# tomoyoshki/focal

Hardware: AMD Instinct MI355X
Metric: pretrain windows/sec (whole node), FOCAL SW_Transformer (higher is better)
Workload: dtype bf16

## Files before the change

focal_amd/_lib.py:

```python
import ctypes as C
import os

_HERE = os.path.dirname(os.path.abspath(__file__))
LIB_PATH = os.environ.get("FOCAL_HIP_LIB") or os.path.join(_HERE, "libfocal_hip.so")

FOCAL_F32, FOCAL_BF16 = 0, 1
ACT_NONE, ACT_GELU, ACT_RELU_OUT = 0, 1, 2
EPI_NONE, EPI_RESIDUAL, EPI_RELU, EPI_GELU = 0, 1, 2, 3
BN_EVAL, BN_TRAIN, BN_PARTIAL, BN_FINALIZE = 0, 1, 2, 3
BN_SCRATCH_ZEROED = 16
BN_STAT_SLOTS = 16
ABI_VERSION = 14


class DropDesc(C.Structure):
    _fields_ = [("rng", C.c_void_p), ("stream_elem", C.c_uint32), ("p_elem", C.c_float),
                ("stream_path", C.c_uint32), ("p_path", C.c_float), ("rows_per_sample", C.c_int)]


class FFTDesc(C.Structure):
    _fields_ = [(n, C.c_int) for n in ("B", "C", "I", "n", "n1", "n2")]


class AugDesc(C.Structure):
# ... 134 lines not shown
    "focal_pad_patch_embed_ape_ln2_fwd": (C.c_int, [C.POINTER(Embed2Desc), P, P, P, P, P, P, P, P, P, C.c_float, C.c_int, P, P, P]),
    "focal_ape_bwd": (C.c_int, [C.c_int, C.c_int, P, P, P]),
    "focal_ape_add_fwd": (C.c_int, [C.c_int, C.c_int, P, P, P]),
    "focal_layernorm_fwd": (C.c_int, [C.POINTER(LNDesc), P, P, P, P, P, P]),
    "focal_layernorm_bwd": (C.c_int, [C.POINTER(LNDesc), P, P, P, P, P, C.c_int, P, P, P, C.POINTER(DropDesc), P]),
    "focal_mask_cast": (C.c_int, [C.c_int, C.c_int, C.c_int, P, C.POINTER(DropDesc), P, P]),
    "focal_linear_fwd": (C.c_int, [C.POINTER(LinearDesc), P, P, P, P, P, P, P]),
    "focal_linear_resid_ln_fwd": (C.c_int, [C.POINTER(LinearDesc), P, P, P, P, P, P, P, C.c_float, P, P, P]),
    "focal_linear_resid_ln_supported": (C.c_int, [C.c_int, C.c_int, C.c_int]),
    "focal_linear_bwd_data": (C.c_int, [C.POINTER(LinearDesc), P, P, P, P, P]),
    "focal_linear_bwd_data_ln": (C.c_int, [C.POINTER(LinearDesc), P, P, P, P, P, P, P, P, P, C.POINTER(DropDesc), P]),
    "focal_linear_bwd_data_ln_supported": (C.c_int, [C.c_int, C.c_int, C.c_int]),
    "focal_linear_bwd_weight": (C.c_int, [C.POINTER(LinearDesc), P, P, P, P, P]),
    "focal_linear_bwd_weight_workgroups": (C.c_int, [C.POINTER(LinearDesc)]),
    "focal_linear_bwd_weight_kernel": (C.c_int, [C.POINTER(LinearDesc)]),
    "focal_linear_bwd_weight_group": (C.c_int, [C.c_int, C.c_int, C.POINTER(DwProblem), P]),
    "focal_linear_bwd_weight_group_supported": (C.c_int, [C.c_int, C.c_int, C.c_int, C.c_int]),
    "focal_linear_bwd_weight_group_workgroups": (C.c_int, [C.c_int, C.c_int, C.POINTER(DwProblem)]),
    "focal_linear_bwd_weight_group_f32": (C.c_int, [C.c_int, C.c_int, C.POINTER(DwProblem), C.c_int, C.c_void_p]),
    "focal_linear_bwd_weight_group_f32_workgroups": (C.c_int, [C.c_int, C.c_int, C.POINTER(DwProblem), C.c_int]),
    "focal_linear_bwd_weight_group_kind": (C.c_int, [C.c_int, C.c_int, C.c_int, C.c_int]),
    "focal_mlp_supported": (C.c_int, [C.c_int, C.c_int, C.c_int]),
    "focal_mlp_fwd": (C.c_int, [C.POINTER(MlpDesc), P, P, P, P, P, P, P, P, P, P, P, P, P]),
    "focal_mlp_bwd": (C.c_int, [C.POINTER(MlpDesc), P, P, P, P, P, P, P, P, P, P, P, P, P, P, P, C.POINTER(DropDesc), P, P, P, P, P]),
    "focal_mlp_bwd_partials_floats": (C.c_long, [C.POINTER(MlpDesc)]),
    "focal_mlp_proj_supported": (C.c_int, [C.c_int, C.c_int, C.c_int]),
    "focal_mlp_proj_fwd": (C.c_int, [C.POINTER(MlpDesc), P, P, P, P, C.POINTER(DropDesc), P, P, P, P, P, P, P, P, P, P, P, P, P, P, P, P]),
    "focal_mlp_wide_supported": (C.c_int, [C.c_int, C.c_int, C.c_int]),
    "focal_mlp_wide_fwd": (C.c_int, [C.POINTER(MlpDesc), P, P, P, P, P, P, P, P, P, P, P, P, P, P]),
    "focal_mlp_wide_proj_supported": (C.c_int, [C.c_int, C.c_int, C.c_int]),
# ... 90 lines not shown
```

focal_amd/csrc/gemm.hpp:

```cpp
#pragma once
#include <stdlib.h>
#include <type_traits>
#include "common.hpp"

enum GemmPro { PRO_NONE = 0, PRO_GELU = 1, PRO_MASK = 2, PRO_CONV = 3 };
enum GemmEpi { EPI_STORE = 0, EPI_RESID = 1, EPI_MUL_AUX = 2, EPI_RELU = 3, EPI_RELU_BWD = 4, EPI_ATOMIC = 5, EPI_GELU_FWD = 6,
               EPI_RESID_LN = 7,
               EPI_LN_BWD = 8,
               EPI_STORE_STATS = 9 };

struct MaskParams {
  const uint32_t* seed;
  uint32_t stream_elem;
  float p_elem;
  uint32_t stream_path;
  float p_path;
  int rows_per_sample;
  int ncols;
};

struct GemmParams {
  int M, N, K;
  const void* A; long lda; long strideA;
  const void* B; long ldb; long strideB;
// ... 284 lines not shown
__global__ __launch_bounds__(256) void focal_dw_tail_group_kernel(const DwTailGroup g) {
  using TA = float;
  using TB = float;
  using TC = float;
  constexpr bool TRA = true, TRB = true;
  constexpr int PROA = PRO_NONE, PROB = PRO_NONE, EPI = EPI_ATOMIC, BM = 64, BN = 64, BKM = 2;
  int pi = 0;
#pragma unroll
  for (int q = 0; q < DW_TAIL_MAX - 1; ++q) pi += (q < g.n - 1 && (int)blockIdx.x >= g.wg_end[q]) ? 1 : 0;
  const int start = pi > 0 ? g.wg_end[pi - 1] : 0;
  const GemmParams& p = g.p[pi];
  const int block = (int)blockIdx.x - start, nblocks = g.wg_end[pi] - start;
#include "gemm_body.inc"
}

static inline void focal_dw_plan(int M, int N, long rows, int target, int* bm_out, int* bn_out, int* splits_out) {
  const int bm = 64, bn = 64;
  const long tiles = (long)((M + bm - 1) / bm) * ((N + bn - 1) / bn);
  const long target_wg = target > 0 ? target : 512;
  long splits = (target_wg + tiles - 1) / tiles;
  const long min_rows = 256;
  const long max_splits = (rows + min_rows - 1) / min_rows;
  if (splits > max_splits) splits = max_splits;
  if (splits < 1) splits = 1;
  *bm_out = bm; *bn_out = bn; *splits_out = (int)splits;
}

static inline bool focal_dw_ring_shape(int M, int N, long rows) {
  return M % 64 == 0 && N % 64 == 0 && rows % 64 == 0 && rows >= 64;
}
// ... 3 lines not shown
  int pairs = (splits + 1) / 2;
  if (tiles <= 256 && tiles * pairs > 256) pairs = 256 / tiles;
  return pairs < 1 ? 1 : pairs;
}

struct GemmSpec {
  int compute;
  int a_dtype, b_dtype, c_dtype;
  bool tra, trb;
  int proA, proB, epi;
};
int focal_launch_gemm_bf16(const GemmSpec& s, const GemmParams& p, hipStream_t stream);
int focal_launch_gemm_f32(const GemmSpec& s, const GemmParams& p, hipStream_t stream);
int focal_launch_dw_tail_bf16(const DwTailGroup& g, hipStream_t stream);
int focal_launch_dw_tail_f32(const DwTailGroup& g, hipStream_t stream);
static inline int focal_launch_gemm(const GemmSpec& s, const GemmParams& p, hipStream_t stream) {
  if ((p.epi.p_elem > 0.f || p.proA.p_elem > 0.f || p.proB.p_elem > 0.f) && ((long)p.M >= (1L << 24) || (long)p.K >= (1L << 24) || (long)p.N >= (1L << 24))) {
    focal_set_error("gemm: a dimension beyond 2^24 with an element mask (MaskEval indexes elements with 24-bit multiplies)");
    return FOCAL_EUNSUPPORTED;
  }
  return s.compute == FOCAL_F32 ? focal_launch_gemm_f32(s, p, stream) : focal_launch_gemm_bf16(s, p, stream);
}
```

focal_amd/csrc/gemm_bf16.hip:

```cpp
#include <stdlib.h>
#include <type_traits>
#include "gemm_ring.hpp"
#include "gemm_dw_ring.hpp"
#define GEMM_CT bf16_t
#define GEMM_TAIL_FN focal_launch_dw_tail_bf16
#define GEMM_FN focal_launch_gemm_bf16
#include "gemm_dispatch.inc"
```

focal_amd/csrc/gemm_body.inc:

```
  using Cfg = GemmCfg<CT>;
  constexpr int BK = Cfg::BK * BKM, KI = Cfg::KI;
  using StA = OperandStage<CT, TA, TRA, PROA, BM, BKM>;
  using StB = OperandStage<CT, TB, TRB, PROB, BN, BKM>;
  using FA = FragLoad<CT, TRA, StA::PITCH>;
  using FB = FragLoad<CT, TRB, StB::PITCH>;
  constexpr int WGN = (BN <= 64) ? 1 : 2, WGM = 4 / WGN;
  constexpr int WR = BM / WGM, WC = BN / WGN;
  constexpr int TM = WR / 16, TN = WC / 16;

  constexpr int OPER_BYTES = (StA::LDS_ELEMS + StB::LDS_ELEMS) * (int)sizeof(CT);
  constexpr int EPI_RP = (WC > 64 || WR < 32) ? 16 : 32;
  constexpr int STAGE_BYTES = 4 * EPI_RP * (WC + 4) * 4;
  constexpr int LDS_BYTES = OPER_BYTES > STAGE_BYTES ? OPER_BYTES : STAGE_BYTES;
  __shared__ __attribute__((aligned(16))) char lds_raw[LDS_BYTES];
  CT* lds = reinterpret_cast<CT*>(lds_raw);
  CT* ldsA = lds;
  CT* ldsB = lds + StA::LDS_ELEMS;

  const int tid = threadIdx.x, lane = tid & 63, wave = tid >> 6;
  const int wm = wave / WGN, wn = wave % WGN;
  const int tiles_n = (p.N + BN - 1) / BN, tiles_m = (p.M + BM - 1) / BM;
  const int ntiles = tiles_m * tiles_n;
  const int logical = xcd_remap(block, nblocks);
  const int tile = logical % ntiles, z = logical / ntiles;
  const int m0 = (tile / tiles_n) * BM, n0 = (tile % tiles_n) * BN;
  const int bz = z / p.splits, sp = z % p.splits;

  const TA* A = reinterpret_cast<const TA*>(p.A) + (long)bz * p.strideA;
  const TB* B = reinterpret_cast<const TB*>(p.B) + (long)bz * p.strideB;
  TC* C = reinterpret_cast<TC*>(p.C) + (long)bz * p.strideC;

  const int KT = (p.K + BK - 1) / BK;
  const int kt_per = (KT + p.splits - 1) / p.splits;
  const int kt0 = sp * kt_per;
  const int kt1 = min(KT, kt0 + kt_per);
  const int k_end = min(p.K, kt1 * BK);

  MaskEval meA, meB, meE;
  if (PROA != PRO_NONE) meA.init(p.proA);
  if (PROB != PRO_NONE) meB.init(p.proB);
  if (EPI == EPI_RESID || EPI == EPI_GELU_FWD || EPI == EPI_RESID_LN) meE.init(p.epi);

  f32x4 acc[TM][TN];
#pragma unroll
  for (int i = 0; i < TM; ++i)
#pragma unroll
    for (int j = 0; j < TN; ++j) acc[i][j] = f32x4{0.f, 0.f, 0.f, 0.f};

  float csum[8] = {0.f, 0.f, 0.f, 0.f, 0.f, 0.f, 0.f, 0.f};
  const bool do_colsum = TRA && (p.colsumA != nullptr) && (n0 == 0);

  constexpr bool PF2 = false;
  StA sa0, sa1;
  StB sb0, sb1;
  auto step = [&](StA& sa, StB& sb, int kt, int kt_next) {
    if (TRA && do_colsum) sa.template store<true>(ldsA, m0, kt * BK, tid, meA, csum);
// ... 109 lines not shown
        const int row = rr + lane / LPR;
        const int m = mbase + row;
        if (m >= p.M || n >= p.N) continue;
        float v[CPL];
        loadN<CPL>(stage + row * WPITCH + c, v);
#pragma unroll
        for (int e = 0; e < CPL; ++e) v[e] += bias[e];
        TC* dst = C + (long)m * p.ldc + n;
        if (EPI == EPI_STORE) {
          storeN<CPL>(dst, v);
        } else if (EPI == EPI_STORE_STATS) {
          storeN<CPL>(dst, v);
          if constexpr (CPL == 4) {
#pragma unroll
            for (int e = 0; e < 4; ++e) { st_s[e] += v[e]; st_q[e] += v[e] * v[e]; }
          }
        } else if (EPI == EPI_RESID) {
          float r[CPL];
          loadN<CPL>(p.resid + (long)m * p.ldr + n, r);
          const float rowm = meE.row_mult(m);
#pragma unroll
          for (int e = 0; e < CPL; ++e) v[e] = r[e] + v[e] * rowm * meE.elem_mult(m, n + e);
          storeN<CPL>(dst, v);
        } else if (EPI == EPI_RESID_LN) {
          float r[CPL];
          loadN<CPL>(p.resid + (long)m * p.ldr + n, r);
          const float rowm = meE.row_mult(m);
#pragma unroll
          for (int e = 0; e < CPL; ++e) v[e] = r[e] + v[e] * rowm * meE.elem_mult(m, n + e);
          storeN<CPL>(dst, v);
// ... 117 lines not shown
```

focal_amd/csrc/gemm_dispatch.inc:

```

#define GEMM_LAUNCH(BM_, BN_, BKM_)                                                                                         \
  do {                                                                                                                      \
    dim3 grid(ceil_div(p.M, BM_) * ceil_div(p.N, BN_) * nz);                                                                \
    focal_note_kernel("focal_gemm_kernel<%s, trA=%d, trB=%d, proA=%d, proB=%d, epi=%d, %dx%d>", sizeof(CT) == 2 ? "bf16" : "f32", (int)TRA, (int)TRB, PA, PB, EPI, BM_, BN_); \
    FOCAL_LAUNCH((focal_gemm_kernel<CT, TA, TB, TC, TRA, TRB, PA, PB, EPI, BM_, BN_, BKM_>), grid, dim3(256), 0, stream, p); \
  } while (0)

template <typename CT, typename TA, typename TB, typename TC, bool TRA, bool TRB, int PA, int PB, int EPI>
static int launch_dw(GemmParams p, long rows, hipStream_t stream) {
  int bm, bn, splits;
  focal_dw_plan(p.M, p.N, rows, p.dw_target, &bm, &bn, &splits);
  p.splits = splits;
  if constexpr (std::is_same<CT, bf16_t>::value && std::is_same<TA, bf16_t>::value && std::is_same<TB, bf16_t>::value &&
                PA == PRO_NONE && PB == PRO_NONE) {
    const bool aligned = ((uintptr_t)p.A % 16 == 0) && ((uintptr_t)p.B % 16 == 0) && (p.lda % 8 == 0) && (p.ldb % 8 == 0);
    if (aligned && p.batch == 1 && bm == 64 && bn == 64 && focal_dw_ring_shape(p.M, p.N, rows)) {
      hipError_t e;
      if (p.splits >= 2) {
        p.splits = focal_dw_ring_pairs(p.M, p.N, p.splits);
        focal_note_kernel("focal_dw_ring_kernel<64, 4, 2>");
        e = focal_launch_dw_ring<64, 4, 2>(p, stream);
      } else {
        focal_note_kernel("focal_dw_ring_kernel<64, 4, 1>");
        e = focal_launch_dw_ring<64, 4, 1>(p, stream);
// ... 99 lines not shown
          focal_set_error("gemm (pipelined, LayerNorm epilogue): launch failed: %s", hipGetErrorString(e));
          return FOCAL_EHIP;
        }
        return FOCAL_OK;
      }
    }
    if (p.N != 64 || p.splits != 1 || p.batch != 1) {
      focal_set_error("gemm: the residual + LayerNorm epilogue needs N == 64, or bf16 operands with N == 128 / 256 and K %% 64 == 0 (got N = %d, K = %d)", p.N, p.K);
      return FOCAL_EUNSUPPORTED;
    }
    const int nz = 1;
    GEMM_LAUNCH(64, 64, 1);
    FOCAL_LAUNCH_CHECK();
    return FOCAL_OK;
  }
  const long min_wg = 512;
  const long z = (long)p.batch * p.splits;
  const int nz = p.batch * p.splits;
  bool narrow_n = (p.N % 128 != 0) || (p.N < 128);
  bool small_m = (p.M % 128 != 0 && p.M < 1024) || (p.M <= 256);
  if (!small_m && !narrow_n && (long)ceil_div(p.M, 128) * ceil_div(p.N, 128) * z < min_wg) narrow_n = true;
  if (!small_m && narrow_n && (long)ceil_div(p.M, 128) * ceil_div(p.N, 64) * z < min_wg) small_m = true;
  if (!std::is_same<CT, float>::value && p.K <= 1024) small_m = true;
  if (!narrow_n && !small_m) GEMM_LAUNCH(128, 128, 1);
  else if (!small_m) GEMM_LAUNCH(128, 64, 1);
  else GEMM_LAUNCH(64, 64, 1);
  FOCAL_LAUNCH_CHECK();
  return FOCAL_OK;
}

#define GEMM_TRY(AF32, BF32, CF32, TRA_, TRB_, PA_, PB_, EPI_)                                                          \
  if (s.a_dtype == ((AF32) ? FOCAL_F32 : ct_code) && s.b_dtype == ((BF32) ? FOCAL_F32 : ct_code) &&                     \
      s.c_dtype == ((CF32) ? FOCAL_F32 : ct_code) && s.tra == (TRA_) && s.trb == (TRB_) && s.proA == (PA_) &&            \
      s.proB == (PB_) && s.epi == (EPI_))                                                                               \
    return launch_tiles<GEMM_CT, std::conditional<(AF32), float, GEMM_CT>::type,                                        \
                        std::conditional<(BF32), float, GEMM_CT>::type, std::conditional<(CF32), float, GEMM_CT>::type, \
                        (TRA_), (TRB_), (PA_), (PB_), (EPI_)>(p, stream);

int GEMM_FN(const GemmSpec& s, const GemmParams& p, hipStream_t stream) {
  const int ct_code = std::is_same<GEMM_CT, float>::value ? FOCAL_F32 : FOCAL_BF16;
// ... 12 lines not shown
  GEMM_TRY(true, false, true, false, true, PRO_NONE, PRO_NONE, EPI_RELU_BWD)
  GEMM_TRY(true, false, true, false, true, PRO_NONE, PRO_NONE, EPI_STORE)
  GEMM_TRY(false, false, true, true, true, PRO_NONE, PRO_NONE, EPI_ATOMIC)
  GEMM_TRY(true, false, true, true, true, PRO_MASK, PRO_NONE, EPI_ATOMIC)
  GEMM_TRY(true, true, true, true, true, PRO_NONE, PRO_NONE, EPI_ATOMIC)
  GEMM_TRY(false, false, true, false, false, PRO_CONV, PRO_NONE, EPI_STORE)
  GEMM_TRY(false, false, true, false, false, PRO_CONV, PRO_NONE, EPI_STORE_STATS)
  GEMM_TRY(false, false, true, false, false, PRO_CONV, PRO_NONE, EPI_RESID)
  GEMM_TRY(false, false, true, true, true, PRO_NONE, PRO_CONV, EPI_ATOMIC)
  focal_set_error("gemm: unsupported combination a=%d b=%d c=%d trA=%d trB=%d proA=%d proB=%d epi=%d (compute %d)",
                  s.a_dtype, s.b_dtype, s.c_dtype, (int)s.tra, (int)s.trb, s.proA, s.proB, s.epi, ct_code);
  return FOCAL_EUNSUPPORTED;
}
#undef GEMM_TRY

int GEMM_TAIL_FN(const DwTailGroup& g, hipStream_t stream) {
  if (g.n <= 0) return FOCAL_OK;
  focal_note_kernel("focal_dw_tail_group_kernel<%s>", sizeof(GEMM_CT) == 2 ? "bf16" : "f32");
  FOCAL_LAUNCH((focal_dw_tail_group_kernel<GEMM_CT>), dim3(g.wg_end[g.n - 1]), dim3(256), 0, stream, g);
  FOCAL_LAUNCH_CHECK();
  return FOCAL_OK;
}
```

focal_amd/csrc/gemm_f32.hip:

```cpp
#include <stdlib.h>
#include <type_traits>
#include "gemm_ring.hpp"
#include "gemm_dw_ring.hpp"
#define GEMM_CT float
#define GEMM_TAIL_FN focal_launch_dw_tail_f32
#define GEMM_FN focal_launch_gemm_f32
#include "gemm_dispatch.inc"
```

focal_amd/csrc/linear.hip:

```cpp
#include <stdlib.h>
#include "gemm.hpp"
#include "gemm_dw_group.hpp"
#include "gemm_dw_ring.hpp"
#include "gemm_ring.hpp"

static MaskParams to_mask(const focal_drop_desc& d, int ncols) {
  MaskParams m;
  m.seed = d.rng;
  m.stream_elem = d.stream_elem;
  m.p_elem = d.p_elem;
  m.stream_path = d.stream_path;
  m.p_path = d.p_path;
  m.rows_per_sample = d.rows_per_sample;
  m.ncols = ncols;
  return m;
}
static MaskParams no_mask() {
  MaskParams m;
  memset(&m, 0, sizeof(m));
  return m;
}

static int check_desc(const focal_linear_desc* d) {
  FOCAL_CHECK_ARG(d != nullptr, "linear: null descriptor");
// ... 202 lines not shown
  if (ring && splits >= 2) splits = focal_dw_ring_pairs(d->N, d->K, splits);
  *wgs = ((d->N + bm - 1) / bm) * ((d->K + bn - 1) / bn) * splits;
  return true;
}

extern "C" int focal_linear_bwd_weight_workgroups(const focal_linear_desc* d) {
  int kernel, wgs;
  return dw_launch_plan(d, &kernel, &wgs) ? wgs : 0;
}

extern "C" int focal_linear_bwd_weight_kernel(const focal_linear_desc* d) {
  int kernel, wgs;
  return dw_launch_plan(d, &kernel, &wgs) ? kernel : 0;
}

static bool dw_group_fits(const focal_dw_problem& q) {
  return q.M > 0 && q.N > 0 && q.K > 0 && q.M % 64 == 0 && q.N % 128 == 0 && q.K % 128 == 0 && q.dy && q.x && q.dw &&
         ((uintptr_t)q.dy % 16 == 0) && ((uintptr_t)q.x % 16 == 0) && ((uintptr_t)q.dw % 16 == 0);
}

extern "C" int focal_linear_bwd_weight_group_supported(int dtype, int M, int N, int K) {
  return dtype == FOCAL_BF16 && M > 0 && M % 64 == 0 && N % 128 == 0 && K % 128 == 0;
}

static int dw_group_build(int dtype, int n, const focal_dw_problem* probs, DwGroupParams* gp, int* wgs) {
  FOCAL_CHECK_ARG(dtype == FOCAL_BF16, "linear_bwd_weight_group: bf16 operands only (dtype %d)", dtype);
  FOCAL_CHECK_ARG(n >= 1 && n <= DWG_MAX_PROBLEMS && probs, "linear_bwd_weight_group: 1 .. %d problems (got %d)", DWG_MAX_PROBLEMS, n);
  memset(gp, 0, sizeof(*gp));
  gp->nprob = n;
  for (int i = 0; i < n; ++i) {
// ... 120 lines not shown
```

focal_amd/ops.py:

```python
import ctypes as C
import math
import os

import torch

from . import _lib
from ._lib import (ACT_GELU, ACT_NONE, ACT_RELU_OUT, EPI_GELU, EPI_NONE, EPI_RELU, EPI_RESIDUAL, FOCAL_BF16, FOCAL_F32,
                   AdamWDesc, AttnDesc, BNDesc, ConvDesc, ConvInDesc, DropDesc, Embed2Desc, EmbedDesc, FFTDesc, GRUDesc, LinearDesc,
                   LNDesc, LossDesc, MlpDesc, check)

_TORCH2CODE = {torch.float32: FOCAL_F32, torch.bfloat16: FOCAL_BF16}
_CODE2TORCH = {v: k for k, v in _TORCH2CODE.items()}


def code(dtype):
    return _TORCH2CODE[dtype]


def torch_dtype(c):
    return _CODE2TORCH[c]


def _stream():
    return torch.cuda.current_stream().cuda_stream
# ... 474 lines not shown
    return bool(_lib.load().focal_linear_bwd_data_ln_supported(dtype_code, N, K))


def linear_bwd_data_ln(d, dy, w, ln_x, ln_stats, ln_gamma, g, dgamma, dbeta, g_masked=None, mask=None):
    _need_cuda(dy, w, ln_x, ln_stats, ln_gamma, g, dgamma, dbeta, g_masked)
    if g_masked is not None:
        mask = mask or NO_DROP
    check(_lib.load().focal_linear_bwd_data_ln(C.byref(d), _p(dy), _p(w), _p(ln_x), _p(ln_stats), _p(ln_gamma), _p(g), _p(dgamma), _p(dbeta),
                                               _p(g_masked), C.byref(mask) if mask is not None else None, _stream()))


def linear_bwd_weight(d, dy, x, dw, dbias):
    check(_lib.load().focal_linear_bwd_weight(C.byref(d), _p(dy), _p(x), _p(dw), _p(dbias), _stream()))


def dw_group_supported(dtype_code, M, N, K):
    return bool(_lib.load().focal_linear_bwd_weight_group_supported(dtype_code, M, N, K))


def dw_group_kind(dtype_code, M, N, K):
    return int(_lib.load().focal_linear_bwd_weight_group_kind(dtype_code, M, N, K))


def _dw_problems(items, exclusive):
    arr = (_lib.DwProblem * len(items))()
    for i, (dy, x, dw, db) in enumerate(items):
        _need_cuda(dy, x, dw, db)
        arr[i] = _lib.DwProblem(_p(dy), _p(x), _p(dw), _p(db), dy.shape[0], dy.shape[1], x.shape[1], 1 if exclusive else 0)
    return arr

# ... 583 lines not shown
```

focal_amd/src/models/SW_Transformer.py:

```python
import os
import sys

import torch
import torch.nn as nn

_ROOT = os.path.abspath(os.path.join(os.path.dirname(__file__), "..", "..", ".."))
if _ROOT not in sys.path:
    sys.path.insert(0, _ROOT)

from focal_amd import runtime
from focal_amd.backbone import HipBackbone, run_stage
from focal_amd.head_engine import ClassifierHead
from focal_amd.loc_engine import LocFusionStage, run_loc_stage
from focal_amd.swin_engine import ProjectorHead, SwinModEncoder
from input_utils.padding_utils import get_padded_size
from models.FusionModules import LocContextLayer, TransformerFusionBlock
from models.SwinModules import BasicLayer, PatchEmbed, PatchMerging


class SW_Transformer(HipBackbone):
    def __init__(self, args) -> None:
        super().__init__()
        self.args = args
        self.config = args.dataset_config["SW_Transformer"]
        self.modalities = args.dataset_config["modality_names"]
        self.locations = args.dataset_config["location_names"]
        self.num_segments = args.dataset_config["num_segments"]
        self.drop_rate = self.config["dropout_ratio"]
        self.attn_drop_rate = self.config["attn_drop_rate"]
# ... 71 lines not shown
            self.mod_projectors[mod] = nn.Sequential(nn.Linear(cfg["loc_out_channels"], out_dim), nn.ReLU(),
                                                     nn.Linear(out_dim, out_dim))
        self.mod_fusion_layers = TransformerFusionBlock(cfg["loc_out_channels"], cfg["loc_head_num"],
                                                        cfg["dropout_ratio"], cfg["dropout_ratio"])
        self.sample_dim = cfg["loc_out_channels"]
        n_cls = dcfg[self.args.task]["num_classes"]
        if self.args.train_mode == "supervised" or cfg["pretrained_head"] == "linear":
            self.class_layer = nn.Sequential(nn.Linear(self.sample_dim, n_cls))
        else:
            self.class_layer = nn.Sequential(nn.Linear(self.sample_dim, cfg["fc_dim"]), nn.GELU(), nn.Linear(cfg["fc_dim"], n_cls))
        M = len(self.modalities)
        self._encoders = {(loc, mod): SwinModEncoder(self, loc, mod, li * M + mi)
                          for li, loc in enumerate(self.locations) for mi, mod in enumerate(self.modalities)}
        self._loc_stages = ({mod: LocFusionStage(self, mod, mi) for mi, mod in enumerate(self.modalities)}
                            if len(self.locations) > 1 else {})
        self._heads = {mod: ProjectorHead(self, mod) for mod in self.modalities}
        self._class_head = ClassifierHead(self, "mod_fusion_layers", cfg["loc_head_num"], cfg["dropout_ratio"])

    def forward_encoder(self, freq_x, class_head=True, proj_head=False, defer_join=False):
        if class_head:
            return self.forward_classifier(freq_x)
        loc = self.locations[0]
        view = self._fwd_calls
        self._fwd_calls = (self._fwd_calls + 1) & 0xFFFF
        dev = next(self.parameters()).device
        if dev.type != "cuda":
            from focal_amd._lib import FocalHipError
            raise FocalHipError("the FOCAL HIP path needs the model on a ROCm device (no CPU fallback)")
        cur = torch.cuda.current_stream(dev)
        out = {}
        self.arena()
# ... 47 lines not shown
```

focal_amd/swin_engine.py:

```python
import os
from typing import NamedTuple

import torch

from . import ops
from ._lib import ACT_GELU, ACT_NONE, EPI_GELU, EPI_NONE, EPI_RESIDUAL


def tail_fp32(bb, which="mod_in"):
    if bb.compute_dtype == torch.float32:
        return False
    sel = os.environ.get("FOCAL_TAIL_FP32", "projector")
    return sel == "both" or sel == which


def tail_weight(bb, ar, name, which="mod_in"):
    return ar.master(name) if tail_fp32(bb, which) else ar.operand(name)


class BlockPlan(NamedTuple):
    attn_qkv: bool
    mlp: str
    proj: str
    next_ln: bool
# ... 205 lines not shown
        pool = self.__dict__.setdefault("_mlp_ws", {})
        n = ops.mlp_bwd_partials_floats(d_mlp)
        ws = pool.get((n, dev))
        if ws is None:
            ws = pool[(n, dev)] = torch.empty(n, dtype=torch.float32, device=dev)
        return ws

    def backward(self, saved, dfeat):
        bb, ar = self.bb, self.bb.arena()
        ct = bb.compute_dtype
        dev = dfeat.device
        if dfeat.dtype != torch.float32 or not dfeat.is_contiguous():
            dfeat = dfeat.float().contiguous()
        pin, d_in, xf = saved["pin"], saved["d_in"], saved["x_final"]
        d_in_b = ops.linear_desc(d_in.dtype, d_in.M, d_in.N, d_in.K, d_in.x_dtype, d_in.y_dtype)
        ops.linear_bwd_weight(d_in_b, dfeat, xf, ar.g(f"{pin}.weight"), ar.g(f"{pin}.bias"))
        g = torch.empty_like(xf)
        ops.linear_bwd_data(d_in_b, dfeat, tail_weight(bb, ar, f"{pin}.weight"), None, g)
        blocks = saved["blocks"]
        last = blocks[-1]
        gm = ops.mask_cast(g.view(last["M"], last["C"]), last["d_fc2"].out_drop, ct)
        stop = 0
        if getattr(bb, "split_backward", False) and saved["merges"] and saved.get("embed") is None:
            stop = max(m["after_block"] for m in saved["merges"])
        state = dict(g=g, gm=gm, next=len(blocks) - 1)
        self._backward_blocks(saved, state, stop)
        if stop > 0:
            saved["_resume"] = state
            bb.pending_backward.append((self, saved, torch.cuda.current_stream(dev)))
            return
        self._backward_tail(saved, state)

    def backward_rest(self, saved):
        state = saved.pop("_resume")
        self._backward_blocks(saved, state, 0)
        self._backward_tail(saved, state)
# ... 147 lines not shown
        z = torch.empty(B, E, dtype=torch.float32, device=feat.device)
        ops.linear_fwd(d2, h, tail_weight(bb, ar, f"{self.pre}.2.weight", "projector"), ar.master(f"{self.pre}.2.bias"), None, z)
        return z, dict(feat=feat, h=h, d0=d0, d2=d2)

    def backward(self, saved, dz):
        ar = self.bb.arena()
        if dz.dtype != torch.float32 or not dz.is_contiguous():
            dz = dz.float().contiguous()
        ops.linear_bwd_weight(saved["d2"], dz, saved["h"], ar.g(f"{self.pre}.2.weight"), ar.g(f"{self.pre}.2.bias"))
        dh = torch.empty_like(saved["h"])
        ops.linear_bwd_data(saved["d2"], dz, tail_weight(self.bb, ar, f"{self.pre}.2.weight", "projector"), saved["h"], dh)
        ops.linear_bwd_weight(saved["d0"], dh, saved["feat"], ar.g(f"{self.pre}.0.weight"), ar.g(f"{self.pre}.0.bias"))
        dfeat = torch.empty_like(saved["feat"])
        ops.linear_bwd_data(saved["d0"], dh, tail_weight(self.bb, ar, f"{self.pre}.0.weight", "projector"), None, dfeat)
        return dfeat
```

include/focal_hip.h:

```cpp
#ifndef FOCAL_HIP_H
#define FOCAL_HIP_H

#include <stddef.h>
#include <stdint.h>

#ifdef __cplusplus
extern "C" {
#endif

#define FOCAL_ABI_VERSION 14

enum { FOCAL_OK = 0, FOCAL_EINVAL = -1, FOCAL_EUNSUPPORTED = -2, FOCAL_EWORKSPACE = -3, FOCAL_EHIP = -4 };
enum { FOCAL_F32 = 0, FOCAL_BF16 = 1 };

int focal_abi_version(void);
const char* focal_last_kernel(void);
const char* focal_last_error(void);

enum { FOCAL_TRACE_DISPATCH = 1, FOCAL_TRACE_EVENTS = 2 };
typedef struct {
  char kernel[384];
  unsigned grid[3], block[3];
  void* stream;
  float us;
// ... 113 lines not shown
int focal_linear_fwd(const focal_linear_desc* d, const void* x, const void* w, const float* bias, const float* resid,
                     void* y, void* act_grad, void* stream);
int focal_linear_resid_ln_fwd(const focal_linear_desc* d, const void* x, const void* w, const float* bias, const float* resid,
                              float* y, const float* gamma, const float* beta, float eps, void* y_ln, float* stats, void* stream);
int focal_linear_resid_ln_supported(int dtype, int N, int K);
int focal_linear_bwd_data(const focal_linear_desc* d, const void* dy, const void* w, const void* x, void* dx,
                          void* stream);
int focal_linear_bwd_data_ln(const focal_linear_desc* d, const void* dy, const void* w, const float* ln_x, const float* ln_stats,
                             const float* ln_gamma, float* g, float* dgamma, float* dbeta, void* g_masked, const focal_drop_desc* mask,
                             void* stream);
int focal_linear_bwd_data_ln_supported(int dtype, int N, int K);
int focal_linear_bwd_weight(const focal_linear_desc* d, const void* dy, const void* x, float* dw, float* dbias,
                            void* stream);
int focal_linear_bwd_weight_workgroups(const focal_linear_desc* d);
int focal_linear_bwd_weight_kernel(const focal_linear_desc* d);

#define FOCAL_DW_GROUP_MAX_PROBLEMS 20
typedef struct {
  const void* dy; const void* x; float* dw; float* dbias;
  int M, N, K;
  int exclusive;
} focal_dw_problem;
int focal_linear_bwd_weight_group(int dtype, int n, const focal_dw_problem* problems, void* stream);
int focal_linear_bwd_weight_group_supported(int dtype, int M, int N, int K);
int focal_linear_bwd_weight_group_kind(int dtype, int M, int N, int K);
int focal_linear_bwd_weight_group_workgroups(int dtype, int n, const focal_dw_problem* problems);
int focal_linear_bwd_weight_group_f32(int compute, int n, const focal_dw_problem* problems, int workgroups, void* stream);
int focal_linear_bwd_weight_group_f32_workgroups(int compute, int n, const focal_dw_problem* problems, int workgroups);

typedef struct { int dtype; int M, C, hidden; focal_drop_desc drop_hidden, drop_out; float ln_eps; } focal_mlp_desc;
// ... 150 lines not shown
```

Baseline: 51540.

## Fuse tail linear weight- and data-gradient GEMMs into one paired launch with mask-cast epilogue

Adds a combined kernel that runs the weight-gradient GEMM (split-K atomic) and the data-gradient GEMM in one grid, with blocks partitioned between the two, sharing one LDS buffer. A new epilogue writes dx and also the dropout-masked cast copy, which removes the separate mask_cast pass. It is used for the encoder's final projection backward and for the projector head's two linears. This cuts kernel launches and lets the two small GEMMs fill the GPU together, at the cost of a larger shared LDS allocation that may lower occupancy.

```diff
diff --git a/focal_amd/_lib.py b/focal_amd/_lib.py
--- a/focal_amd/_lib.py
+++ b/focal_amd/_lib.py
@@ -172,6 +172,9 @@
     "focal_linear_bwd_weight": (C.c_int, [C.POINTER(LinearDesc), P, P, P, P, P]),
     "focal_linear_bwd_weight_workgroups": (C.c_int, [C.POINTER(LinearDesc)]),
     "focal_linear_bwd_weight_kernel": (C.c_int, [C.POINTER(LinearDesc)]),
+    "focal_linear_bwd_pair_supported": (C.c_int, [C.POINTER(LinearDesc), C.c_int]),
+    "focal_linear_bwd_pair_workgroups": (C.c_int, [C.POINTER(LinearDesc)]),
+    "focal_linear_bwd_pair": (C.c_int, [C.POINTER(LinearDesc), P, P, P, P, P, P, P, C.c_int, C.POINTER(DropDesc), C.c_int, P]),
     "focal_linear_bwd_weight_group": (C.c_int, [C.c_int, C.c_int, C.POINTER(DwProblem), P]),
     "focal_linear_bwd_weight_group_supported": (C.c_int, [C.c_int, C.c_int, C.c_int, C.c_int]),
     "focal_linear_bwd_weight_group_workgroups": (C.c_int, [C.c_int, C.c_int, C.POINTER(DwProblem)]),
diff --git a/focal_amd/csrc/gemm.hpp b/focal_amd/csrc/gemm.hpp
--- a/focal_amd/csrc/gemm.hpp
+++ b/focal_amd/csrc/gemm.hpp
@@ -7,7 +7,8 @@
 enum GemmEpi { EPI_STORE = 0, EPI_RESID = 1, EPI_MUL_AUX = 2, EPI_RELU = 3, EPI_RELU_BWD = 4, EPI_ATOMIC = 5, EPI_GELU_FWD = 6,
                EPI_RESID_LN = 7,
                EPI_LN_BWD = 8,
-               EPI_STORE_STATS = 9 };
+               EPI_STORE_STATS = 9,
+               EPI_STORE_MASKCAST = 10 };
 
 struct MaskParams {
   const uint32_t* seed;
@@ -322,6 +323,52 @@
 #include "gemm_body.inc"
 }
 
+struct TailPair { int dw_wgs; GemmParams dw, dx; };
+template <typename CT, bool TRA, bool TRB, int BM, int BN, int BKM> constexpr int gemm_body_lds_bytes() {
+  constexpr int WGN = (BN <= 64) ? 1 : 2, WGM = 4 / WGN, WR = BM / WGM, WC = BN / WGN;
+  constexpr int oper = (OperandStage<CT, CT, TRA, PRO_NONE, BM, BKM>::LDS_ELEMS + OperandStage<CT, CT, TRB, PRO_NONE, BN, BKM>::LDS_ELEMS) * (int)sizeof(CT);
+  constexpr int stage = 4 * ((WC > 64 || WR < 32) ? 16 : 32) * (WC + 4) * 4;
+  return oper > stage ? oper : stage;
+}
+template <typename CT, int EPI_DX>
+__global__ __launch_bounds__(256) void focal_tail_pair_kernel(const TailPair g) {
+  constexpr int DW_LDS = gemm_body_lds_bytes<CT, true, true, 64, 64, 2>(), DX_LDS = gemm_body_lds_bytes<CT, false, true, 64, 64, 1>();
+  constexpr int GEMM_BODY_SHARED_LDS_BYTES = DW_LDS > DX_LDS ? DW_LDS : DX_LDS;
+  __shared__ __attribute__((aligned(16))) char pair_lds[GEMM_BODY_SHARED_LDS_BYTES];
+#define GEMM_BODY_SHARED_LDS pair_lds
+  if ((int)blockIdx.x < g.dw_wgs) {
+    using TA = float;
+    using TB = float;
+    using TC = float;
+    constexpr bool TRA = true, TRB = true;
+    constexpr int PROA = PRO_NONE, PROB = PRO_NONE, EPI = EPI_ATOMIC, BM = 64, BN = 64, BKM = 2;
+    const GemmParams& p = g.dw;
+    const int block = (int)blockIdx.x, nblocks = g.dw_wgs;
+#include "gemm_body.inc"
+  } else {
+    using TA = float;
+    using TB = CT;
+    using TC = float;
+    constexpr bool TRA = false, TRB = true;
+    constexpr int PROA = PRO_NONE, PROB = PRO_NONE, EPI = EPI_DX, BM = 64, BN = 64, BKM = 1;
+    const GemmParams& p = g.dx;
+    const int block = (int)blockIdx.x - g.dw_wgs, nblocks = (int)gridDim.x - g.dw_wgs;
+#include "gemm_body.inc"
+  }
+#undef GEMM_BODY_SHARED_LDS
+}
+
+static inline void focal_tile_plan(bool f32_compute, int M, int N, int K, long z, int* bm_out, int* bn_out) {
+  const long min_wg = 512;
+  bool narrow_n = (N % 128 != 0) || (N < 128);
+  bool small_m = (M % 128 != 0 && M < 1024) || (M <= 256);
+  if (!small_m && !narrow_n && (long)((M + 127) / 128) * ((N + 127) / 128) * z < min_wg) narrow_n = true;
+  if (!small_m && narrow_n && (long)((M + 127) / 128) * ((N + 63) / 64) * z < min_wg) small_m = true;
+  if (!f32_compute && K <= 1024) small_m = true;
+  *bm_out = small_m ? 64 : 128;
+  *bn_out = (!narrow_n && !small_m) ? 128 : 64;
+}
+
 static inline void focal_dw_plan(int M, int N, long rows, int target, int* bm_out, int* bn_out, int* splits_out) {
   const int bm = 64, bn = 64;
   const long tiles = (long)((M + bm - 1) / bm) * ((N + bn - 1) / bn);
@@ -355,6 +402,8 @@
 int focal_launch_gemm_f32(const GemmSpec& s, const GemmParams& p, hipStream_t stream);
 int focal_launch_dw_tail_bf16(const DwTailGroup& g, hipStream_t stream);
 int focal_launch_dw_tail_f32(const DwTailGroup& g, hipStream_t stream);
+int focal_launch_tail_pair_bf16(const TailPair& g, int epi_dx, int dx_wgs, hipStream_t stream);
+int focal_launch_tail_pair_f32(const TailPair& g, int epi_dx, int dx_wgs, hipStream_t stream);
 static inline int focal_launch_gemm(const GemmSpec& s, const GemmParams& p, hipStream_t stream) {
   if ((p.epi.p_elem > 0.f || p.proA.p_elem > 0.f || p.proB.p_elem > 0.f) && ((long)p.M >= (1L << 24) || (long)p.K >= (1L << 24) || (long)p.N >= (1L << 24))) {
     focal_set_error("gemm: a dimension beyond 2^24 with an element mask (MaskEval indexes elements with 24-bit multiplies)");
diff --git a/focal_amd/csrc/gemm_bf16.hip b/focal_amd/csrc/gemm_bf16.hip
--- a/focal_amd/csrc/gemm_bf16.hip
+++ b/focal_amd/csrc/gemm_bf16.hip
@@ -4,5 +4,6 @@
 #include "gemm_dw_ring.hpp"
 #define GEMM_CT bf16_t
 #define GEMM_TAIL_FN focal_launch_dw_tail_bf16
+#define GEMM_PAIR_FN focal_launch_tail_pair_bf16
 #define GEMM_FN focal_launch_gemm_bf16
 #include "gemm_dispatch.inc"
diff --git a/focal_amd/csrc/gemm_body.inc b/focal_amd/csrc/gemm_body.inc
--- a/focal_amd/csrc/gemm_body.inc
+++ b/focal_amd/csrc/gemm_body.inc
@@ -12,7 +12,12 @@
   constexpr int EPI_RP = (WC > 64 || WR < 32) ? 16 : 32;
   constexpr int STAGE_BYTES = 4 * EPI_RP * (WC + 4) * 4;
   constexpr int LDS_BYTES = OPER_BYTES > STAGE_BYTES ? OPER_BYTES : STAGE_BYTES;
+#ifdef GEMM_BODY_SHARED_LDS
+  static_assert(LDS_BYTES <= GEMM_BODY_SHARED_LDS_BYTES, "the including kernel's shared buffer is too small for this body");
+  char* const lds_raw = GEMM_BODY_SHARED_LDS;
+#else
   __shared__ __attribute__((aligned(16))) char lds_raw[LDS_BYTES];
+#endif
   CT* lds = reinterpret_cast<CT*>(lds_raw);
   CT* ldsA = lds;
   CT* ldsB = lds + StA::LDS_ELEMS;
@@ -39,7 +44,7 @@
   MaskEval meA, meB, meE;
   if (PROA != PRO_NONE) meA.init(p.proA);
   if (PROB != PRO_NONE) meB.init(p.proB);
-  if (EPI == EPI_RESID || EPI == EPI_GELU_FWD || EPI == EPI_RESID_LN) meE.init(p.epi);
+  if (EPI == EPI_RESID || EPI == EPI_GELU_FWD || EPI == EPI_RESID_LN || EPI == EPI_STORE_MASKCAST) meE.init(p.epi);
 
   f32x4 acc[TM][TN];
 #pragma unroll
@@ -179,6 +184,16 @@
           if constexpr (CPL == 4) {
 #pragma unroll
             for (int e = 0; e < 4; ++e) { st_s[e] += v[e]; st_q[e] += v[e] * v[e]; }
+          }
+        } else if (EPI == EPI_STORE_MASKCAST) {
+          storeN<CPL>(dst, v);
+          if constexpr (CPL == 4) {
+            const long off = (long)m * p.ldc + n;
+            const uint32_t trow = (uint32_t)(off / meE.ncols);
+            const float pm = meE.on_p ? drop_mult(meE.p, meE.rps > 1 ? __umulhi(trow, meE.rps_magic) : trow) : 1.0f;
+#pragma unroll
+            for (int e = 0; e < CPL; ++e) v[e] *= meE.on_e ? pm * drop_mult(meE.e, (uint32_t)off + e) : pm;
+            storeN<CPL>(reinterpret_cast<CT*>(p.aux_out) + off, v);
           }
         } else if (EPI == EPI_RESID) {
           float r[CPL];
diff --git a/focal_amd/csrc/gemm_dispatch.inc b/focal_amd/csrc/gemm_dispatch.inc
--- a/focal_amd/csrc/gemm_dispatch.inc
+++ b/focal_amd/csrc/gemm_dispatch.inc
@@ -137,16 +137,11 @@
     FOCAL_LAUNCH_CHECK();
     return FOCAL_OK;
   }
-  const long min_wg = 512;
-  const long z = (long)p.batch * p.splits;
   const int nz = p.batch * p.splits;
-  bool narrow_n = (p.N % 128 != 0) || (p.N < 128);
-  bool small_m = (p.M % 128 != 0 && p.M < 1024) || (p.M <= 256);
-  if (!small_m && !narrow_n && (long)ceil_div(p.M, 128) * ceil_div(p.N, 128) * z < min_wg) narrow_n = true;
-  if (!small_m && narrow_n && (long)ceil_div(p.M, 128) * ceil_div(p.N, 64) * z < min_wg) small_m = true;
-  if (!std::is_same<CT, float>::value && p.K <= 1024) small_m = true;
-  if (!narrow_n && !small_m) GEMM_LAUNCH(128, 128, 1);
-  else if (!small_m) GEMM_LAUNCH(128, 64, 1);
+  int bm, bn;
+  focal_tile_plan(std::is_same<CT, float>::value, p.M, p.N, p.K, (long)p.batch * p.splits, &bm, &bn);
+  if (bm == 128 && bn == 128) GEMM_LAUNCH(128, 128, 1);
+  else if (bm == 128) GEMM_LAUNCH(128, 64, 1);
   else GEMM_LAUNCH(64, 64, 1);
   FOCAL_LAUNCH_CHECK();
   return FOCAL_OK;
@@ -189,6 +184,20 @@
 }
 #undef GEMM_TRY
 
+int GEMM_PAIR_FN(const TailPair& g, int epi_dx, int dx_wgs, hipStream_t stream) {
+  const dim3 grid(g.dw_wgs + dx_wgs);
+  focal_note_kernel("focal_tail_pair_kernel<%s, dX epi=%d>", sizeof(GEMM_CT) == 2 ? "bf16" : "f32", epi_dx);
+  if (epi_dx == EPI_STORE) FOCAL_LAUNCH((focal_tail_pair_kernel<GEMM_CT, EPI_STORE>), grid, dim3(256), 0, stream, g);
+  else if (epi_dx == EPI_RELU_BWD) FOCAL_LAUNCH((focal_tail_pair_kernel<GEMM_CT, EPI_RELU_BWD>), grid, dim3(256), 0, stream, g);
+  else if (epi_dx == EPI_STORE_MASKCAST) FOCAL_LAUNCH((focal_tail_pair_kernel<GEMM_CT, EPI_STORE_MASKCAST>), grid, dim3(256), 0, stream, g);
+  else {
+    focal_set_error("tail pair: no data-gradient epilogue %d", epi_dx);
+    return FOCAL_EUNSUPPORTED;
+  }
+  FOCAL_LAUNCH_CHECK();
+  return FOCAL_OK;
+}
+
 int GEMM_TAIL_FN(const DwTailGroup& g, hipStream_t stream) {
   if (g.n <= 0) return FOCAL_OK;
   focal_note_kernel("focal_dw_tail_group_kernel<%s>", sizeof(GEMM_CT) == 2 ? "bf16" : "f32");
diff --git a/focal_amd/csrc/gemm_f32.hip b/focal_amd/csrc/gemm_f32.hip
--- a/focal_amd/csrc/gemm_f32.hip
+++ b/focal_amd/csrc/gemm_f32.hip
@@ -4,5 +4,6 @@
 #include "gemm_dw_ring.hpp"
 #define GEMM_CT float
 #define GEMM_TAIL_FN focal_launch_dw_tail_f32
+#define GEMM_PAIR_FN focal_launch_tail_pair_f32
 #define GEMM_FN focal_launch_gemm_f32
 #include "gemm_dispatch.inc"
diff --git a/focal_amd/csrc/linear.hip b/focal_amd/csrc/linear.hip
--- a/focal_amd/csrc/linear.hip
+++ b/focal_amd/csrc/linear.hip
@@ -240,6 +240,81 @@
   return dw_launch_plan(d, &kernel, &wgs) ? kernel : 0;
 }
 
+static bool pair_fits(const focal_linear_desc* d, int gm_dtype) {
+  if (d == nullptr || d->M <= 0 || d->N <= 0 || d->K <= 0) return false;
+  if (d->dtype != FOCAL_F32 && d->dtype != FOCAL_BF16) return false;
+  const int ec = d->dtype == FOCAL_BF16 ? 8 : 4;
+  if (d->N % ec != 0 || d->K % ec != 0) return false;
+  if (d->x_dtype != FOCAL_F32 || d->y_dtype != FOCAL_F32 || d->epilogue == FOCAL_EPI_RESIDUAL) return false;
+  if (d->act_in != FOCAL_ACT_NONE && d->act_in != FOCAL_ACT_RELU_OUT) return false;
+  if (gm_dtype >= 0 && (gm_dtype != d->dtype || d->act_in != FOCAL_ACT_NONE)) return false;
+  int bm, bn;
+  focal_tile_plan(d->dtype == FOCAL_F32, d->M, d->K, d->N, 1, &bm, &bn);
+  return bm == 64 && bn == 64;
+}
+
+extern "C" int focal_linear_bwd_pair_supported(const focal_linear_desc* d, int gm_dtype) { return pair_fits(d, gm_dtype) ? 1 : 0; }
+
+static int pair_dx_workgroups(const focal_linear_desc* d) { return ceil_div(d->M, 64) * ceil_div(d->K, 64); }
+
+extern "C" int focal_linear_bwd_pair_workgroups(const focal_linear_desc* d) {
+  if (!pair_fits(d, -1)) return 0;
+  return focal_linear_bwd_weight_workgroups(d) + pair_dx_workgroups(d);
+}
+
+extern "C" int focal_linear_bwd_pair(const focal_linear_desc* d, const void* dy, const void* w, const void* x, void* dx, float* dw,
+                                     float* dbias, void* gm, int gm_dtype, const focal_drop_desc* mask, int mask_cols, void* stream) {
+  if (int rc = check_desc(d)) return rc;
+  FOCAL_CHECK_ARG(dy && w && x && dx && dw, "linear_bwd_pair: null tensor");
+  if (!pair_fits(d, gm ? gm_dtype : -1)) {
+    focal_set_error("linear_bwd_pair: unsupported layer (dtype %d, M=%d N=%d K=%d, x/y dtype %d/%d, act_in %d, epilogue %d, masked copy dtype %d): "
+                    "fp32 activations, no output mask, a 64 x 64 data-gradient tile and a masked copy in the compute type only",
+                    d->dtype, d->M, d->N, d->K, d->x_dtype, d->y_dtype, d->act_in, d->epilogue, gm ? gm_dtype : -1);
+    return FOCAL_EUNSUPPORTED;
+  }
+  FOCAL_CHECK_ARG(gm || !mask, "linear_bwd_pair: mask without a masked copy");
+  if (gm) {
+    FOCAL_CHECK_ARG(mask_cols > 0 && mask_cols % 4 == 0 && ((long)d->M * d->K) % mask_cols == 0,
+                    "linear_bwd_pair: dx [%d, %d] is not a whole number of %d-column token rows", d->M, d->K, mask_cols);
+    const long token_rows = (long)d->M * d->K / mask_cols;
+    FOCAL_CHECK_ARG((long)d->M * d->K < (1L << 32) && (!mask || mask->rows_per_sample <= 1 || token_rows * (long)mask->rows_per_sample < (1L << 32)),
+                    "linear_bwd_pair: %ld token rows exceed the mask's 32-bit arithmetic", token_rows);
+  }
+  TailPair g;
+  memset(&g, 0, sizeof(g));
+  {
+    GemmParams& p = g.dw;
+    p.M = d->N; p.N = d->K; p.K = d->M;
+    p.A = dy; p.lda = d->N;
+    p.B = x; p.ldb = d->K;
+    p.C = dw; p.ldc = d->K;
+    p.batch = 1; p.alpha = 1.f;
+    p.dw_target = d->dw_workgroups;
+    p.colsumA = dbias;
+    int bm, bn, splits;
+    focal_dw_plan(p.M, p.N, p.K, p.dw_target, &bm, &bn, &splits);
+    p.splits = splits;
+    g.dw_wgs = ceil_div(p.M, bm) * ceil_div(p.N, bn) * splits;
+  }
+  {
+    GemmParams& p = g.dx;
+    p.M = d->M; p.N = d->K; p.K = d->N;
+    p.A = dy; p.lda = d->N;
+    p.B = w; p.ldb = d->K;
+    p.C = dx; p.ldc = d->K;
+    p.batch = 1; p.splits = 1; p.alpha = 1.f;
+    p.aux = x; p.ldaux = d->K;
+    p.aux_out = gm;
+    focal_drop_desc dd;
+    memset(&dd, 0, sizeof(dd));
+    if (mask) dd = *mask;
+    p.epi = gm ? to_mask(dd, mask_cols) : no_mask();
+  }
+  const int epi = gm ? EPI_STORE_MASKCAST : d->act_in == FOCAL_ACT_RELU_OUT ? EPI_RELU_BWD : EPI_STORE;
+  return d->dtype == FOCAL_F32 ? focal_launch_tail_pair_f32(g, epi, pair_dx_workgroups(d), (hipStream_t)stream)
+                               : focal_launch_tail_pair_bf16(g, epi, pair_dx_workgroups(d), (hipStream_t)stream);
+}
+
 static bool dw_group_fits(const focal_dw_problem& q) {
   return q.M > 0 && q.N > 0 && q.K > 0 && q.M % 64 == 0 && q.N % 128 == 0 && q.K % 128 == 0 && q.dy && q.x && q.dw &&
          ((uintptr_t)q.dy % 16 == 0) && ((uintptr_t)q.x % 16 == 0) && ((uintptr_t)q.dw % 16 == 0);
diff --git a/focal_amd/ops.py b/focal_amd/ops.py
--- a/focal_amd/ops.py
+++ b/focal_amd/ops.py
@@ -512,6 +512,23 @@
     check(_lib.load().focal_linear_bwd_weight(C.byref(d), _p(dy), _p(x), _p(dw), _p(dbias), _stream()))
 
 
+def linear_bwd_pair_supported(d, gm_dtype=None):
+    return bool(_lib.load().focal_linear_bwd_pair_supported(C.byref(d), -1 if gm_dtype is None else code(gm_dtype)))
+
+
+def linear_bwd_pair_workgroups(d):
+    return int(_lib.load().focal_linear_bwd_pair_workgroups(C.byref(d)))
+
+
+def linear_bwd_pair(d, dy, w, x, dx, dw, dbias, gm=None, mask=None):
+    _need_cuda(dy, w, x, dx, dw, dbias, gm)
+    if gm is not None and gm.numel() != dx.numel():
+        raise _lib.FocalHipError("linear_bwd_pair: gm must cover dx")
+    check(_lib.load().focal_linear_bwd_pair(C.byref(d), _p(dy), _p(w), _p(x), _p(dx), _p(dw), _p(dbias), _p(gm),
+                                            -1 if gm is None else code(gm.dtype), C.byref(mask) if mask is not None else None,
+                                            0 if gm is None else gm.shape[-1], _stream()))
+
+
 def dw_group_supported(dtype_code, M, N, K):
     return bool(_lib.load().focal_linear_bwd_weight_group_supported(dtype_code, M, N, K))
 
diff --git a/focal_amd/src/models/SW_Transformer.py b/focal_amd/src/models/SW_Transformer.py
--- a/focal_amd/src/models/SW_Transformer.py
+++ b/focal_amd/src/models/SW_Transformer.py
@@ -12,7 +12,7 @@
 from focal_amd.backbone import HipBackbone, run_stage
 from focal_amd.head_engine import ClassifierHead
 from focal_amd.loc_engine import LocFusionStage, run_loc_stage
-from focal_amd.swin_engine import ProjectorHead, SwinModEncoder
+from focal_amd.swin_engine import SwinModEncoder, SwinProjectorHead
 from input_utils.padding_utils import get_padded_size
 from models.FusionModules import LocContextLayer, TransformerFusionBlock
 from models.SwinModules import BasicLayer, PatchEmbed, PatchMerging
@@ -114,7 +114,7 @@
                           for li, loc in enumerate(self.locations) for mi, mod in enumerate(self.modalities)}
         self._loc_stages = ({mod: LocFusionStage(self, mod, mi) for mi, mod in enumerate(self.modalities)}
                             if len(self.locations) > 1 else {})
-        self._heads = {mod: ProjectorHead(self, mod) for mod in self.modalities}
+        self._heads = {mod: SwinProjectorHead(self, mod) for mod in self.modalities}
         self._class_head = ClassifierHead(self, "mod_fusion_layers", cfg["loc_head_num"], cfg["dropout_ratio"])
 
     def forward_encoder(self, freq_x, class_head=True, proj_head=False, defer_join=False):
diff --git a/focal_amd/swin_engine.py b/focal_amd/swin_engine.py
--- a/focal_amd/swin_engine.py
+++ b/focal_amd/swin_engine.py
@@ -243,12 +243,17 @@
             dfeat = dfeat.float().contiguous()
         pin, d_in, xf = saved["pin"], saved["d_in"], saved["x_final"]
         d_in_b = ops.linear_desc(d_in.dtype, d_in.M, d_in.N, d_in.K, d_in.x_dtype, d_in.y_dtype)
-        ops.linear_bwd_weight(d_in_b, dfeat, xf, ar.g(f"{pin}.weight"), ar.g(f"{pin}.bias"))
         g = torch.empty_like(xf)
-        ops.linear_bwd_data(d_in_b, dfeat, tail_weight(bb, ar, f"{pin}.weight"), None, g)
         blocks = saved["blocks"]
         last = blocks[-1]
-        gm = ops.mask_cast(g.view(last["M"], last["C"]), last["d_fc2"].out_drop, ct)
+        if ops.linear_bwd_pair_supported(d_in_b, ct):
+            gm = torch.empty(last["M"], last["C"], dtype=ct, device=dev)
+            ops.linear_bwd_pair(d_in_b, dfeat, tail_weight(bb, ar, f"{pin}.weight"), xf.view(d_in_b.M, d_in_b.K), g, ar.g(f"{pin}.weight"),
+                                ar.g(f"{pin}.bias"), gm=gm, mask=last["d_fc2"].out_drop)
+        else:
+            ops.linear_bwd_weight(d_in_b, dfeat, xf, ar.g(f"{pin}.weight"), ar.g(f"{pin}.bias"))
+            ops.linear_bwd_data(d_in_b, dfeat, tail_weight(bb, ar, f"{pin}.weight"), None, g)
+            gm = ops.mask_cast(g.view(last["M"], last["C"]), last["d_fc2"].out_drop, ct)
         stop = 0
         if getattr(bb, "split_backward", False) and saved["merges"] and saved.get("embed") is None:
             stop = max(m["after_block"] for m in saved["merges"])
@@ -426,3 +431,20 @@
         dfeat = torch.empty_like(saved["feat"])
         ops.linear_bwd_data(saved["d0"], dh, tail_weight(self.bb, ar, f"{self.pre}.0.weight", "projector"), None, dfeat)
         return dfeat
+
+
+class SwinProjectorHead(ProjectorHead):
+
+    def backward(self, saved, dz):
+        ar = self.bb.arena()
+        d2, d0 = saved["d2"], saved["d0"]
+        if not (ops.linear_bwd_pair_supported(d2) and ops.linear_bwd_pair_supported(d0)):
+            return super().backward(saved, dz)
+        if dz.dtype != torch.float32 or not dz.is_contiguous():
+            dz = dz.float().contiguous()
+        w = lambda i: tail_weight(self.bb, ar, f"{self.pre}.{i}.weight", "projector")
+        dh = torch.empty_like(saved["h"])
+        ops.linear_bwd_pair(d2, dz, w(2), saved["h"], dh, ar.g(f"{self.pre}.2.weight"), ar.g(f"{self.pre}.2.bias"))
+        dfeat = torch.empty_like(saved["feat"])
+        ops.linear_bwd_pair(d0, dh, w(0), saved["feat"], dfeat, ar.g(f"{self.pre}.0.weight"), ar.g(f"{self.pre}.0.bias"))
+        return dfeat
diff --git a/include/focal_hip.h b/include/focal_hip.h
--- a/include/focal_hip.h
+++ b/include/focal_hip.h
@@ -151,6 +151,10 @@
                             void* stream);
 int focal_linear_bwd_weight_workgroups(const focal_linear_desc* d);
 int focal_linear_bwd_weight_kernel(const focal_linear_desc* d);
+int focal_linear_bwd_pair_supported(const focal_linear_desc* d, int gm_dtype);
+int focal_linear_bwd_pair_workgroups(const focal_linear_desc* d);
+int focal_linear_bwd_pair(const focal_linear_desc* d, const void* dy, const void* w, const void* x, void* dx, float* dw, float* dbias,
+                          void* gm, int gm_dtype, const focal_drop_desc* mask, int mask_cols, void* stream);
 
 #define FOCAL_DW_GROUP_MAX_PROBLEMS 20
 typedef struct {
```

After: 52050 (median of 6 runs). No clear change (+1.0%).
